# tsereda/fast-cwdm

Hardware: AMD Instinct MI355X
Metric: denoising-steps/sec on 8-ch 128^3 volumes (1000-step DDPM, i2i cWDM) (higher is better)
Workload: dtype bf16; 1 GPU; config2: BraTS 3->1 conditional synthesis, 1xMI355X per replica, 128^3 subbands, 1000-step DDPM (direct linear schedule); model=UNetModel run.sh (mc 64, mult 1,2,2,4,4, 2 res blocks, 81.5M params), global_batch=1, seq_len=2097152, parallelism=replicas1

## Files before the change

### fast-cwdm_amd/csrc/conv3d_sg.hip

```cpp
#include <algorithm>
#include <atomic>
#include <cstdlib>
#include <type_traits>

#include "conv3d_v4.hpp"

namespace cwdm {

typedef float sg_f32x4 __attribute__((ext_vector_type(4)));

template <int BX, int BY, int PAD>
struct SGCfg {
  static constexpr int HX = BX + 2 * PAD, HY = BY + 2 * PAD, HZ = 4 + 2 * PAD, HV = HX * HY * HZ;
  static constexpr int PCS = (HV + 63) / 64;
  static constexpr int HVP = PCS * 64;
  static constexpr int SUB = HVP * 32;
  static constexpr int BUF = 2 * SUB;
  static constexpr int WBUF = 27 * 1024;
  static constexpr int SMEM = 2 * BUF + 2 * WBUF;
  static constexpr int LPO = 16 / BX;
  static constexpr int NR = 3 * LPO + 3;
  static_assert(BX * BY == 64, "a brick plane is 64 voxels");
};

struct SGParams {
  V4Params v;
  int ntile16;
  int parts;
  int tx, ty;
  int ksplit, kper;
  float* part;
  unsigned* count;
  int xcd;
  int diag;
  int late;
};
#ifdef CWDM_SG_DIAG
#define SG_DIAG(bit) ((q.diag & (bit)) != 0)
#else
#define SG_DIAG(bit) false
#endif

thread_local unsigned* g_sg_sync = nullptr;
constexpr int64_t kSgSyncWords = 1 << 16;

__device__ __forceinline__ void sg_mfma(sg_f32x4& acc, const u32x4& a, const u32x4& b, bf16_t*) {
  acc = __builtin_amdgcn_mfma_f32_16x16x32_bf16(__builtin_bit_cast(bf16x8, a), __builtin_bit_cast(bf16x8, b), acc, 0,
                                                0, 0);
}
__device__ __forceinline__ void sg_mfma(sg_f32x4& acc, const u32x4& a, const u32x4& b, f16_t*) {
  acc = __builtin_amdgcn_mfma_f32_16x16x32_f16(__builtin_bit_cast(f16x8, a), __builtin_bit_cast(f16x8, b), acc, 0, 0,
                                               0);
}

template <typename T, int BX, int BY, int MODE, int TAPS>
__global__ void __launch_bounds__(256) conv3d_sg_kernel(SGParams q) {
  static_assert(TAPS == 27 || TAPS == 1, "3x3x3 or 1x1");
  constexpr int PAD = TAPS == 27 ? 1 : 0;
  using C = SGCfg<BX, BY, PAD>;
  const V4Params& p = q.v;
  __shared__ __attribute__((aligned(1024))) unsigned char smem[C::SMEM];
  const int tid = threadIdx.x, lane = tid & 63, l16 = lane & 15, kq = lane >> 4;
  const int wv = __builtin_amdgcn_readfirstlane(tid >> 6);
  V4_STAMP(0);
#ifdef CWDM_CONV_STAMPS
  if (p.stamps && tid == 0) {
    p.stamps[(long long)blockIdx.x * 24 + 20] = __builtin_amdgcn_s_memrealtime();
    p.stamps[(long long)blockIdx.x * 24 + 22] = __builtin_amdgcn_s_getreg((4 << 0) | (0 << 6) | (31 << 11));
    p.stamps[(long long)blockIdx.x * 24 + 23] = __builtin_amdgcn_s_getreg((20 << 0) | (0 << 6) | (31 << 11));
  }
#endif

  int wi = blockIdx.x;
  if (q.xcd) {
    const int n = (int)gridDim.x, xj = wi & 7, q8 = n >> 3, r8 = n & 7;
    wi = (xj < r8 ? xj * (q8 + 1) : r8 * (q8 + 1) + (xj - r8) * q8) + (wi >> 3);
  }
  const int t16 = wi % q.ntile16;
  const int ks = (wi / q.ntile16) % q.ksplit;
  const int st = wi / (q.ntile16 * q.ksplit);
  const int b = st / q.parts, brick = st - b * q.parts;
  const int tx = q.tx, ty = q.ty;
  const int x0 = (brick % tx) * BX, y0 = ((brick / tx) % ty) * BY, z0 = (brick / (tx * ty)) * 4;
  const int SH = MODE == 1 ? p.H >> 1 : p.H, SW = MODE == 1 ? p.W >> 1 : p.W;
  const int nch = p.nch / 2;
  const int cb0 = ks * q.kper, cb1 = min(nch, cb0 + q.kper);

  auto issue_halo = [&](int c, int hbuf) {
    if (SG_DIAG(2)) return;
    unsigned char* hb = smem + hbuf * C::BUF;
#pragma unroll
    for (int j = 0; j < C::PCS; ++j) {
      const int pc = wv + 4 * j;
      const int sub = pc / (2 * C::PCS), blk = pc - sub * (2 * C::PCS);
      const int hv = blk * 32 + (lane >> 1);
      const int qd = 2 * sub + (lane & 1);
      if (hv >= C::HV) continue;
      int sv = -1;
// ... 8 lines not shown
      const int sc = 2 * c + (qd >> 1);
      const bool s0 = sc < p.nch0;
      const unsigned char* base = s0 ? reinterpret_cast<const unsigned char*>(p.a0) + (long long)b * p.a0_bstride
                                     : reinterpret_cast<const unsigned char*>(p.a1) + (long long)b * p.a1_bstride;
      const __amdgpu_buffer_rsrc_t rs =
          __builtin_amdgcn_make_buffer_rsrc((void*)base, (short)0, (int)(s0 ? p.a0_bytes : p.a1_bytes), 0x00020000);
      const bool cm = s0 && p.a0_cm;
      const unsigned rowb = cm ? 32u : (unsigned)(s0 ? p.ac0 : p.ac1) * 2u;
      const unsigned cofs = cm ? (unsigned)sc * (unsigned)p.a0_cvox * 32u : (unsigned)((s0 ? sc : sc - p.nch0) * 32);
      const unsigned voff = sv >= 0 ? (unsigned)sv * rowb + cofs + (unsigned)((qd & 1) * 16) : 0xFFFFFFF0u;
      __builtin_amdgcn_raw_ptr_buffer_load_lds(rs, (__attribute__((address_space(3))) void*)(hb + pc * 1024), 16, voff,
                                               0, 0, 0);
    }
  };

  const int ct64 = t16 >> 2, row = (t16 & 3) * 16 + l16;
  const unsigned wlane = (unsigned)(row * 32 + (((kq & 1) ^ ((row >> 3) & 1)) << 4));
  const __amdgpu_buffer_rsrc_t wrs = __builtin_amdgcn_make_buffer_rsrc(
      (void*)(p.aw + (long long)ct64 * p.nch * TAPS * 2048), (short)0, p.nch * TAPS * 2048, 0x00020000);
  auto issue_w = [&](int c, int wbuf) {
    if (SG_DIAG(4)) return;
    unsigned char* wb = smem + 2 * C::BUF + wbuf * C::WBUF;
    const unsigned cb = (unsigned)((2 * c + (kq >> 1)) * TAPS) * 2048u + wlane;
#pragma unroll
    for (int j = 0; j < (TAPS + 3) / 4; ++j) {
      const int t = wv + 4 * j;
      if (t < TAPS)
        __builtin_amdgcn_raw_ptr_buffer_load_lds(wrs, (__attribute__((address_space(3))) void*)(wb + t * 1024), 16,
                                                 cb + (unsigned)t * 2048u, 0, 0, 0);
    }
  };

  const int xl = l16 % BX, yl = l16 / BX;
  const int hlane = (kq >> 1) * C::SUB + (kq & 1) * 16 + ((wv * C::HY + yl) * C::HX + xl) * 32;

  sg_f32x4 acc[4];
  {
    float bi[4];
#pragma unroll
    for (int i = 0; i < 4; ++i)
      bi[i] = (p.bias && q.ksplit == 1 && !SG_DIAG(32)) ? p.bias[(long long)b * p.bias_bs + t16 * 16 + 4 * kq + i] : 0.f;
#pragma unroll
    for (int m = 0; m < 4; ++m) acc[m] = sg_f32x4{bi[0], bi[1], bi[2], bi[3]};
  }

  issue_halo(cb0, 0);
  issue_w(cb0, 0);
  asm volatile("s_waitcnt vmcnt(0)" ::: "memory");
  __builtin_amdgcn_s_barrier();
  V4_STAMP(1);
  for (int c = cb0; c < cb1; ++c) {
    const bool has_next = c + 1 < cb1;
    const int buf = (c - cb0) & 1;
    const unsigned char* hb = smem + buf * C::BUF + hlane;
    const unsigned char* wb = smem + 2 * C::BUF + buf * C::WBUF + lane * 16;
    u32x4 av[2][C::NR], aw[2][3];
    auto read_group = [&](u32x4 (&a)[C::NR], u32x4 (&w)[3], int g) {
      if (SG_DIAG(8)) return;
      const int dz = g / 3, dx = g % 3;
#pragma unroll
      for (int dy = 0; dy < 3; ++dy) w[dy] = *reinterpret_cast<const u32x4*>(wb + (dz * 9 + dy * 3 + dx) * 1024);
#pragma unroll
      for (int s = 0; s < C::NR; ++s)
        a[s] = *reinterpret_cast<const u32x4*>(hb + ((dz * C::HY + s) * C::HX + dx) * 32);
    };
    if constexpr (TAPS == 27) {
      read_group(av[0], aw[0], 0);
    } else {
#pragma unroll
      for (int s2 = 0; s2 < 4 * C::LPO; s2 += C::LPO)
        av[0][s2] = *reinterpret_cast<const u32x4*>(hb + s2 * C::HX * 32);
      aw[0][0] = *reinterpret_cast<const u32x4*>(wb);
    }
    const int late = TAPS == 27 ? q.late : 0;
    if (has_next && late == 0) {
      issue_halo(c + 1, buf ^ 1);
      issue_w(c + 1, buf ^ 1);
    }
    if constexpr (TAPS == 27) {
#pragma unroll
      for (int g = 0; g < 9; ++g) {
        if (g + 1 < 9) read_group(av[(g + 1) & 1], aw[(g + 1) & 1], g + 1);
        __builtin_amdgcn_sched_barrier(0);
#pragma unroll
        for (int dy = 0; dy < 3; ++dy)
#pragma unroll
          for (int m = 0; m < 4; ++m)
            if (!SG_DIAG(1)) sg_mfma(acc[m], aw[g & 1][dy], av[g & 1][m * C::LPO + dy], (T*)nullptr);
        __builtin_amdgcn_sched_barrier(0);
        if (has_next && late == g + 1) {
          issue_halo(c + 1, buf ^ 1);
          issue_w(c + 1, buf ^ 1);
        }
      }
    } else {
#pragma unroll
      for (int m = 0; m < 4; ++m) sg_mfma(acc[m], aw[0][0], av[0][m * C::LPO], (T*)nullptr);
    }
    if (has_next) {
      asm volatile("s_waitcnt vmcnt(0)" ::: "memory");
      __builtin_amdgcn_s_barrier();
    }
    if (c - cb0 < 8) V4_STAMP(4 + c - cb0);
  }
  V4_STAMP(12);
  if (SG_DIAG(16)) return;

  if (q.ksplit > 1 && !SG_DIAG(64)) {
    const int tile = st * q.ntile16 + t16;
    const __amdgpu_buffer_rsrc_t prs = __builtin_amdgcn_make_buffer_rsrc(
        q.part + (long long)tile * q.ksplit * 4096, (short)0, q.ksplit * 4096 * 4, 0x00020000);
    const unsigned lofs = (unsigned)(wv * 4 * 64 + lane) * 16u;
#pragma unroll
    for (int m = 0; m < 4; ++m)
      __builtin_amdgcn_raw_buffer_store_b128(__builtin_bit_cast(u32x4, acc[m]), prs,
                                             (unsigned)ks * 16384u + lofs + (unsigned)m * 1024u, 0, 16);
    asm volatile("s_waitcnt vmcnt(0)" ::: "memory");
    __syncthreads();
    unsigned* flag = reinterpret_cast<unsigned*>(smem);
    if (tid == 0)
      *flag = __hip_atomic_fetch_add(&q.count[tile], 1u, __ATOMIC_RELAXED, __HIP_MEMORY_SCOPE_AGENT);
    __syncthreads();
    V4_STAMP(13);
    if (*flag != (unsigned)(q.ksplit - 1)) {
      V4_STAMP(15);
#ifdef CWDM_CONV_STAMPS
      if (p.stamps && tid == 0) p.stamps[(long long)blockIdx.x * 24 + 21] = __builtin_amdgcn_s_memrealtime();
#endif
      return;
    }
    if (tid == 0) __hip_atomic_store(&q.count[tile], 0u, __ATOMIC_RELAXED, __HIP_MEMORY_SCOPE_AGENT);
    float bi[4];
#pragma unroll
    for (int i = 0; i < 4; ++i) bi[i] = p.bias ? p.bias[(long long)b * p.bias_bs + t16 * 16 + 4 * kq + i] : 0.f;
#pragma unroll
    for (int m = 0; m < 4; ++m) {
      sg_f32x4 sum = __builtin_bit_cast(sg_f32x4, __builtin_amdgcn_raw_buffer_load_b128(prs, lofs + m * 1024u, 0, 16));
      for (int k = 1; k < q.ksplit; ++k)
        sum += __builtin_bit_cast(sg_f32x4,
                                  __builtin_amdgcn_raw_buffer_load_b128(prs, (unsigned)k * 16384u + lofs + m * 1024u, 0, 16));
      acc[m] = sum + sg_f32x4{bi[0], bi[1], bi[2], bi[3]};
    }
    V4_STAMP(14);
  }

  const int ox = x0 + xl, oz = z0 + wv;
  const long long HW = (long long)p.H * p.W;
  float ssum[4] = {0.f, 0.f, 0.f, 0.f}, ssq[4] = {0.f, 0.f, 0.f, 0.f};
  const int co = t16 * 16 + 4 * kq;
  bool inb[4];
#pragma unroll
  for (int m = 0; m < 4; ++m) inb[m] = ox < p.W && (y0 + m * C::LPO + yl) < p.H && oz < p.D;
  uint2 rq[4];
  float4 rf[4];
  if (p.rmode >= 0) {
#pragma unroll
    for (int m = 0; m < 4; ++m) {
      const int oy = y0 + m * C::LPO + yl;
      long long rvox = ((long long)b * p.D + oz) * HW + (long long)oy * p.W + ox;
      if (p.rmode == 1)
        rvox = (((long long)b * (p.D >> 1) + (oz >> 1)) * (p.H >> 1) + (oy >> 1)) * (p.W >> 1) + (ox >> 1);
      rq[m] = uint2{0u, 0u};
      rf[m] = make_float4(0.f, 0.f, 0.f, 0.f);
      if (inb[m]) {
        if (p.out_f32) rf[m] = *reinterpret_cast<const float4*>(reinterpret_cast<const float*>(p.res) + rvox * p.cout + co);
        else rq[m] = *reinterpret_cast<const uint2*>(reinterpret_cast<const T*>(p.res) + rvox * p.cout + co);
      }
    }
  }
#pragma unroll
  for (int m = 0; m < 4; ++m) {
    const int oy = y0 + m * C::LPO + yl;
    const long long vox = ((long long)b * p.D + oz) * HW + (long long)oy * p.W + ox;
    float v[4];
#pragma unroll
    for (int i = 0; i < 4; ++i) v[i] = acc[m][i];
    if (p.rmode >= 0) {
      if (p.out_f32) {
        v[0] += rf[m].x; v[1] += rf[m].y; v[2] += rf[m].z; v[3] += rf[m].w;
      } else {
        v[0] += lo2f<T>(rq[m].x); v[1] += hi2f<T>(rq[m].x);
        v[2] += lo2f<T>(rq[m].y); v[3] += hi2f<T>(rq[m].y);
      }
    }
    if (inb[m]) {
#pragma unroll
      for (int i = 0; i < 4; ++i) {
        ssum[i] += v[i];
        ssq[i] += v[i] * v[i];
      }
      if (p.out_f32) {
        *reinterpret_cast<float4*>(reinterpret_cast<float*>(p.out) + vox * p.cout + co) = make_float4(v[0], v[1], v[2], v[3]);
      } else {
        uint2 sq;
        sq.x = pack2<T>(v[0], v[1]);
        sq.y = pack2<T>(v[2], v[3]);
        *reinterpret_cast<uint2*>(reinterpret_cast<T*>(p.out) + vox * p.cout + co) = sq;
      }
    }
  }
  if (p.stats) {
#pragma unroll
    for (int i = 0; i < 4; ++i) {
      ssum[i] = row16_sum(ssum[i]);
      ssq[i] = row16_sum(ssq[i]);
    }
    __syncthreads();
    float* R = reinterpret_cast<float*>(smem);
    if (l16 == 0) {
#pragma unroll
      for (int i = 0; i < 4; ++i) {
        R[wv * 32 + 4 * kq + i] = ssum[i];
        R[wv * 32 + 16 + 4 * kq + i] = ssq[i];
      }
    }
    __syncthreads();
    if (tid < 16) {
      float s = 0.f, s2 = 0.f;
#pragma unroll
      for (int w = 0; w < 4; ++w) {
        s += R[w * 32 + tid];
        s2 += R[w * 32 + 16 + tid];
      }
      const long long pidx = ((long long)b * q.parts + brick) * p.cout + t16 * 16 + tid;
      p.stats[pidx * 2 + 0] = s;
      p.stats[pidx * 2 + 1] = s2;
    }
  }
  V4_STAMP(15);
#ifdef CWDM_CONV_STAMPS
  if (p.stamps && tid == 0) p.stamps[(long long)blockIdx.x * 24 + 21] = __builtin_amdgcn_s_memrealtime();
#endif
}

template __global__ void conv3d_sg_kernel<bf16_t, 16, 4, 0, 27>(SGParams);
template __global__ void conv3d_sg_kernel<bf16_t, 16, 4, 1, 27>(SGParams);
template __global__ void conv3d_sg_kernel<bf16_t, 16, 4, 0, 1>(SGParams);
template __global__ void conv3d_sg_kernel<bf16_t, 8, 8, 0, 27>(SGParams);
template __global__ void conv3d_sg_kernel<bf16_t, 8, 8, 1, 27>(SGParams);
template __global__ void conv3d_sg_kernel<bf16_t, 8, 8, 0, 1>(SGParams);
template __global__ void conv3d_sg_kernel<f16_t, 16, 4, 0, 27>(SGParams);
template __global__ void conv3d_sg_kernel<f16_t, 16, 4, 1, 27>(SGParams);
template __global__ void conv3d_sg_kernel<f16_t, 16, 4, 0, 1>(SGParams);
template __global__ void conv3d_sg_kernel<f16_t, 8, 8, 0, 27>(SGParams);
template __global__ void conv3d_sg_kernel<f16_t, 8, 8, 1, 27>(SGParams);
template __global__ void conv3d_sg_kernel<f16_t, 8, 8, 0, 1>(SGParams);

thread_local bool g_sg_fp32x = false;

namespace {
bool sg_shape_ok(const cwdm_conv3d_desc* d) {
  if (g_conv_path.load(std::memory_order_relaxed) == 1) return false;
  if (!dtype_half(d->dtype) || d->accumulate || d->out1 || d->cout % 64) return false;
  if (d->out_dtype != d->dtype && !(d->out_dtype == CWDM_F32 && g_sg_fp32x)) return false;
  return d->W >= 1 && d->W < kWideMinW && d->H >= 1 && d->D >= 1;
}

struct SgGeom { int bx, tx, ty, tz; int64_t parts() const { return (int64_t)tx * ty * tz; } };
SgGeom sg_geom(const cwdm_conv3d_desc* d) {
  const int bx = d->W >= 16 ? 16 : 8, by = 64 / bx;
  return SgGeom{bx, (int)ceil_div(d->W, bx), (int)ceil_div(d->H, by), (int)ceil_div(d->D, 4)};
// ... 21 lines not shown
int sg_split_for(const cwdm_conv3d_desc* d, int cin, bool skip = false) {
  const int64_t parts = sg_geom(d).parts();
  const int64_t tiles = d->B * parts * (d->cout / 16);
  const int nch = cin / 32;
  static const int64_t target3 = env_ll("CWDM_SG_TARGET", 192);
  static const int64_t target1 = env_ll("CWDM_SG_SKIP_TARGET", target3);
  const int64_t target = skip ? target1 : target3;
  if (tiles >= target || nch < 2) return 1;
  int S = (int)std::min<int64_t>((target + tiles - 1) / tiles, nch);
  const int per = (nch + S - 1) / S;
  S = (nch + per - 1) / per;
  return (tiles * S < (1 << 16) && S > 1) ? S : 1;
}
}

int sg_ksplit(const cwdm_conv3d_desc* d) { return sg_eligible(d) ? sg_split_for(d, d->a_c0 + d->a_c1) : 1; }
int64_t ksplit_slice_voxels(const cwdm_conv3d_desc* d) {
  return sg_shape_ok(d) ? sg_geom(d).parts() * 256 : d->D * d->H * d->W;
}
int sg_skip_ksplit(const cwdm_conv3d_desc* d) { return sg_skip_eligible(d) ? sg_split_for(d, d->b_c0 + d->b_c1, true) : 1; }

int64_t sg_sync_bytes(int ksplit) { return ksplit > 1 ? kSgSyncWords * 4 : 0; }
int64_t plan_sync_bytes() { return kSgSyncWords * 4 + kV5AaWords * 4; }
unsigned* plan_aa_counters() { return g_sg_sync ? g_sg_sync + kSgSyncWords : nullptr; }

namespace {
int sg_counters(SGParams& q, void* own, hipStream_t s) {
  q.count = nullptr;
  if (q.ksplit == 1) return CWDM_OK;
  const int64_t tiles = (int64_t)q.v.B * q.parts * q.ntile16;
  CWDM_REQUIRE(tiles <= kSgSyncWords, CWDM_E_UNSUPPORTED, "conv3d (small grid): too many K-split tiles");
  if (g_sg_sync) {
    q.count = g_sg_sync;
    return CWDM_OK;
  }
  CWDM_REQUIRE(own, CWDM_E_INVALID, "conv3d (small grid): K-split counters missing");
  q.count = reinterpret_cast<unsigned*>(own);
  CWDM_HIP(hipMemsetAsync(own, 0, (size_t)((tiles * 4 + 15) & ~15LL), s));
  return CWDM_OK;
}

template <typename T>
void sg_go_t(const SGParams& q, const cwdm_conv3d_desc* d, int taps, hipStream_t s) {
  const dim3 grid((unsigned)(d->B * q.parts * q.ntile16 * q.ksplit));
  const bool w8 = sg_geom(d).bx == 8;
  if (w8 && taps == 1) {
    hipLaunchKernelGGL((conv3d_sg_kernel<T, 8, 8, 0, 1>), grid, dim3(256), 0, s, q);
  } else if (w8) {
    if (q.v.amode == 1) hipLaunchKernelGGL((conv3d_sg_kernel<T, 8, 8, 1, 27>), grid, dim3(256), 0, s, q);
    else hipLaunchKernelGGL((conv3d_sg_kernel<T, 8, 8, 0, 27>), grid, dim3(256), 0, s, q);
  } else if (taps == 1) {
    hipLaunchKernelGGL((conv3d_sg_kernel<T, 16, 4, 0, 1>), grid, dim3(256), 0, s, q);
  } else if (q.v.amode == 1) {
    hipLaunchKernelGGL((conv3d_sg_kernel<T, 16, 4, 1, 27>), grid, dim3(256), 0, s, q);
  } else {
    hipLaunchKernelGGL((conv3d_sg_kernel<T, 16, 4, 0, 27>), grid, dim3(256), 0, s, q);
  }
}

int sg_go(const SGParams& q0, const cwdm_conv3d_desc* d, int taps, double flops, hipStream_t s) {
  static const int xcd_map = env_not0("CWDM_SG_XCD");
  SGParams q = q0;
  q.xcd = xcd_map;
  static const int late = env_int("CWDM_SG_LATE", 4);
  q.late = late < 0 ? 0 : (late > 9 ? 9 : late);
#ifdef CWDM_SG_DIAG
  static const int diag = env_int("CWDM_SG_DIAGMASK", 0);
  q.diag = diag;
#endif
  prof_begin(s);
  if (d->dtype == CWDM_F16) sg_go_t<f16_t>(q, d, taps, s);
  else sg_go_t<bf16_t>(q, d, taps, s);
  prof_end(s, flops);
  CWDM_LAUNCHED();
  return CWDM_OK;
}
}

int sg_launch(const V4Params& v, const cwdm_conv3d_desc* d, void* partial, hipStream_t s) {
  SGParams q{};
  q.v = v;
  q.ntile16 = d->cout / 16;
  const SgGeom gm = sg_geom(d);
  q.parts = (int)gm.parts();
  q.tx = gm.tx; q.ty = gm.ty;
  q.ksplit = sg_ksplit(d);
  q.kper = ((d->a_c0 + d->a_c1) / 32 + q.ksplit - 1) / q.ksplit;
  q.part = reinterpret_cast<float*>(partial);
  CWDM_REQUIRE(q.ksplit == 1 || partial, CWDM_E_INVALID, "conv3d (small grid): K-split scratch missing");
  int rc;
  if ((rc = sg_counters(q, q.ksplit > 1 ? reinterpret_cast<unsigned char*>(partial) +
                                              (int64_t)q.ksplit * d->B * ksplit_slice_voxels(d) * d->cout * 4
                                        : nullptr, s)))
    return rc;
  return sg_go(q, d, 27, 2.0 * d->B * d->D * d->H * d->W * (double)d->cout * 27.0 * (d->a_c0 + d->a_c1), s);
}

int sg_skip_launch(const cwdm_conv3d_desc* d, void* out, void* partial, hipStream_t s) {
  SGParams q{};
  V4Params& p = q.v;
  const int64_t V = d->D * d->H * d->W;
  p.B = (int)d->B; p.D = (int)d->D; p.H = (int)d->H; p.W = (int)d->W;
  p.cout = d->cout; p.nct = d->cout / 64;
  p.nch0 = d->b_c0 / 16; p.nch = (d->b_c0 + d->b_c1) / 16;
  p.a0 = d->b0; p.ac0 = d->b_c0; p.a1 = d->b1; p.ac1 = d->b_c1;
  p.a0_bstride = V * d->b_c0 * 2; p.a1_bstride = V * d->b_c1 * 2;
  p.a0_bytes = (unsigned)(V * d->b_c0 * 2); p.a1_bytes = (unsigned)(V * d->b_c1 * 2);
  p.amode = 0; p.a0_cm = 0; p.a0_cvox = (int)V;
  p.aw = reinterpret_cast<const unsigned char*>(d->b_w);
  p.bias = nullptr; p.res = nullptr; p.rmode = -1;
  p.out = out; p.stats = nullptr;
  p.out_f32 = (d->out_dtype == CWDM_F32) ? 1 : 0;
  q.ntile16 = d->cout / 16;
  const SgGeom gm = sg_geom(d);
  q.parts = (int)gm.parts();
  q.tx = gm.tx; q.ty = gm.ty;
  q.ksplit = sg_skip_ksplit(d);
  q.kper = ((d->b_c0 + d->b_c1) / 32 + q.ksplit - 1) / q.ksplit;
  q.part = reinterpret_cast<float*>(partial);
  CWDM_REQUIRE(q.ksplit == 1 || partial, CWDM_E_INVALID, "conv3d (small grid): K-split scratch missing");
  int rc;
  if ((rc = sg_counters(q, q.ksplit > 1 ? reinterpret_cast<unsigned char*>(partial) +
                                              (int64_t)q.ksplit * d->B * ksplit_slice_voxels(d) * d->cout * 4
                                        : nullptr, s)))
    return rc;
  return sg_go(q, d, 1, 2.0 * d->B * V * (double)d->cout * (d->b_c0 + d->b_c1), s);
}

}
```

### fast-cwdm_amd/cwdm_hip/_lib.py

```python
import ctypes
import os

_HERE = os.path.dirname(os.path.abspath(__file__))
LIB_PATH = os.environ.get("CWDM_LIB", os.path.join(_HERE, "..", "lib", "libcwdm.so"))

CWDM_F32 = 0
CWDM_BF16 = 1
CWDM_F64 = 2
CWDM_F16 = 3

E_INVALID, E_SHAPE, E_HIP, E_WORKSPACE, E_INDEX, E_UNSUPPORTED = -1, -2, -3, -4, -5, -6

i64 = ctypes.c_int64
vp = ctypes.c_void_p
I64x3 = i64 * 3
I64x4 = i64 * 4


class SamplerArgs(ctypes.Structure):
    _fields_ = [
        ("model_out", vp), ("mo_s", I64x3),
        ("x_t", vp), ("xt_s", I64x3),
        ("x_prev", vp), ("xp_s", I64x3),
        ("noise", vp), ("nz_s", I64x3),
# ... 111 lines not shown
    "cwdm_conv3d_parts": (i64, [ctypes.c_int, i64, i64, i64, ctypes.c_int]),
    "cwdm_space_to_depth": (ctypes.c_int, [vp, ctypes.c_int, i64, i64, i64, i64, ctypes.c_int, vp, ctypes.c_int,
                                           ctypes.c_int, vp]),
    "cwdm_conv3d_pack_s2": (ctypes.c_int, [vp, ctypes.c_int, ctypes.c_int, ctypes.c_int, vp, ctypes.c_int, vp]),
    "cwdm_conv3d_s2_fold_dw": (ctypes.c_int, [vp, ctypes.c_int, ctypes.c_int, vp, ctypes.c_int, vp]),
    "cwdm_conv3d_forward": (ctypes.c_int, [ctypes.POINTER(ConvDesc), vp]),
    "cwdm_conv3d_workspace_bytes": (i64, [ctypes.POINTER(ConvDesc)]),
    "cwdm_gn_finalize": (ctypes.c_int, [vp, i64, ctypes.c_int, vp, i64, ctypes.c_int, vp, vp, ctypes.c_int, i64, i64,
                                        ctypes.c_float, vp, vp, vp]),
    "cwdm_gn_silu_pool": (ctypes.c_int, [vp, ctypes.c_int, vp, i64, i64, i64, i64, ctypes.c_int, vp, vp, vp]),
    "cwdm_gn_apply": (ctypes.c_int, [vp, ctypes.c_int, vp, ctypes.c_int, vp, i64, i64, ctypes.c_int, vp, vp]),
    "cwdm_conv3d_set_path": (ctypes.c_int, [ctypes.c_int]),
    "cwdm_debug_v5_grid": (ctypes.c_int, [ctypes.c_int]),
    "cwdm_debug_v5_aa": (ctypes.c_int, [ctypes.c_int]),
    "cwdm_debug_up_phase": (ctypes.c_int, [ctypes.c_int]),
    "cwdm_debug_stats_wg": (i64, [ctypes.c_int]),
    "cwdm_debug_v5_aa_timeout": (ctypes.c_int, [ctypes.c_int, ctypes.c_int]),
    "cwdm_device_status": (ctypes.c_int, [ctypes.c_int]),
    "cwdm_debug_gn_fin_apply": (ctypes.c_int, [vp, i64, ctypes.c_int, vp, i64, ctypes.c_int, vp, vp, ctypes.c_int,
                                               i64, i64, ctypes.c_float, vp, vp, ctypes.c_int, vp, vp, vp, vp]),
    "cwdm_debug_head2": (ctypes.c_int, [ctypes.c_int]),
    "cwdm_debug_pw_lt": (ctypes.c_int, [ctypes.c_int]),
    "cwdm_debug_conv_stamps": (ctypes.c_int, [vp]),
    "cwdm_conv3d_wgrad": (ctypes.c_int, [ctypes.POINTER(WgradDesc), vp]),
    "cwdm_conv3d_wgrad_workspace_bytes": (i64, [ctypes.c_int, ctypes.c_int, ctypes.c_int]),
    "cwdm_gn_silu_bwd_workspace_bytes": (i64, [ctypes.c_int, i64, i64, i64, i64]),
    "cwdm_gn_silu_bwd": (ctypes.c_int, [vp, ctypes.c_int, vp, ctypes.c_int, vp, ctypes.c_int, vp, vp, vp,
                                        ctypes.c_int, i64, i64, i64, i64, ctypes.c_int, vp, ctypes.c_int, vp,
                                        ctypes.c_int, vp, vp, vp, i64, vp]),
    "cwdm_resample_add": (ctypes.c_int, [vp, vp, ctypes.c_int, i64, i64, i64, i64, ctypes.c_int, ctypes.c_int,
# ... 114 lines not shown
```

### include/cwdm.h

```cpp
#ifndef CWDM_H_
#define CWDM_H_

#include <stddef.h>
#include <stdint.h>

#ifdef __cplusplus
extern "C" {
#endif

typedef struct ihipStream_t* cwdm_stream_t;

enum {
  CWDM_F32 = 0,
  CWDM_BF16 = 1,
  CWDM_F64 = 2,
  CWDM_F16 = 3
};

enum {
  CWDM_OK = 0,
  CWDM_E_INVALID = -1,
  CWDM_E_SHAPE = -2,
  CWDM_E_HIP = -3,
  CWDM_E_WORKSPACE = -4,
// ... 135 lines not shown
                     int64_t B, int64_t voxels, float eps,
                     float* scale_shift, float* mean_rstd ,
                     cwdm_stream_t stream);

int cwdm_gn_silu_pool(const void* x, int C, const float* gn, int64_t B, int64_t d, int64_t h, int64_t w,
                      int dtype, void* out_h, void* out_x, cwdm_stream_t stream);

int cwdm_conv3d_set_path(int path);

int cwdm_debug_v5_grid(int n);

int cwdm_debug_v5_aa(int on);

int cwdm_debug_up_phase(int on);

int64_t cwdm_debug_stats_wg(int on);

int cwdm_debug_v5_aa_timeout(int extra, int spin);

enum { CWDM_DEV_E_AA_TIMEOUT = 1 };
int cwdm_device_status(int clear);

int cwdm_debug_gn_fin_apply(const float* stats0, int64_t parts0, int c0, const float* stats1, int64_t parts1,
                            int c1, const float* gamma, const float* beta, int groups, int64_t B, int64_t voxels,
                            float eps, const void* x0, const void* x1, int dtype, float* scale_shift,
                            float* mean_rstd, void* out_cm, cwdm_stream_t stream);

int cwdm_debug_head2(int mode);

int cwdm_debug_pw_lt(int on);
// ... 102 lines not shown
```

Before: 67.56 denoising-steps/s.

## Add wide small-grid conv forms covering two bricks and/or two channel tiles

Templates the small-grid 3x3x3 conv kernel on NB (bricks along y) and NT (16-channel output tiles per workgroup), so one halo fill feeds more output rows and one weight fill feeds more channels. When LDS cannot hold double buffers, it falls back to single buffering with an extra barrier. A host-side cost model picks the form and K-split per layer. It is on by default through CWDM_SG_WIDE. The aim is more MFMA work per LDS fill and fewer, fuller workgroups on small-grid layers, at the cost of more registers (lower occupancy), fewer workgroups, and possible serialization when single-buffered.

Result: no change. 68.03 denoising-steps/s (median of 6 runs) (+0.7%).

```diff
diff --git a/fast-cwdm_amd/csrc/conv3d_sg.hip b/fast-cwdm_amd/csrc/conv3d_sg.hip
--- a/fast-cwdm_amd/csrc/conv3d_sg.hip
+++ b/fast-cwdm_amd/csrc/conv3d_sg.hip
@@ -9,18 +9,25 @@
 
 typedef float sg_f32x4 __attribute__((ext_vector_type(4)));
 
-template <int BX, int BY, int PAD>
+template <int BX, int BY, int PAD, int NB = 1, int NT = 1>
 struct SGCfg {
-  static constexpr int HX = BX + 2 * PAD, HY = BY + 2 * PAD, HZ = 4 + 2 * PAD, HV = HX * HY * HZ;
+  static constexpr int HX = BX + 2 * PAD, HY = BY * NB + 2 * PAD, HZ = 4 + 2 * PAD, HV = HX * HY * HZ;
   static constexpr int PCS = (HV + 63) / 64;
   static constexpr int HVP = PCS * 64;
   static constexpr int SUB = HVP * 32;
   static constexpr int BUF = 2 * SUB;
-  static constexpr int WBUF = 27 * 1024;
-  static constexpr int SMEM = 2 * BUF + 2 * WBUF;
+  static constexpr int WB1 = 27 * 1024;
+  static constexpr int WBUF = NT * WB1;
+  static constexpr int LDS = 160 * 1024;
+  static constexpr int HBN = 2 * BUF + WBUF <= LDS ? 2 : 1;
+  static constexpr int WBN = HBN * BUF + 2 * WBUF <= LDS ? 2 : 1;
+  static constexpr int SMEM = HBN * BUF + WBN * WBUF;
   static constexpr int LPO = 16 / BX;
-  static constexpr int NR = 3 * LPO + 3;
+  static constexpr int NOP = 4 * NB;
+  static constexpr int NR = (NOP - 1) * LPO + 3;
   static_assert(BX * BY == 64, "a brick plane is 64 voxels");
+  static_assert((NB == 1 || NB == 2) && (NT == 1 || NT == 2), "1 or 2 bricks x 1 or 2 channel tiles");
+  static_assert(PAD == 1 || (NB == 1 && NT == 1), "the wide forms are 27-tap only");
 };
 
 struct SGParams {
@@ -28,6 +35,7 @@
   int ntile16;
   int parts;
   int tx, ty;
+  int typ, tparts;
   int ksplit, kper;
   float* part;
   unsigned* count;
@@ -53,11 +61,12 @@
                                                0);
 }
 
-template <typename T, int BX, int BY, int MODE, int TAPS>
+template <typename T, int BX, int BY, int MODE, int TAPS, int NB = 1, int NT = 1>
 __global__ void __launch_bounds__(256) conv3d_sg_kernel(SGParams q) {
   static_assert(TAPS == 27 || TAPS == 1, "3x3x3 or 1x1");
   constexpr int PAD = TAPS == 27 ? 1 : 0;
-  using C = SGCfg<BX, BY, PAD>;
+  using C = SGCfg<BX, BY, PAD, NB, NT>;
+  constexpr int NOP = C::NOP;
   const V4Params& p = q.v;
   __shared__ __attribute__((aligned(1024))) unsigned char smem[C::SMEM];
   const int tid = threadIdx.x, lane = tid & 63, l16 = lane & 15, kq = lane >> 4;
@@ -79,9 +88,10 @@
   const int t16 = wi % q.ntile16;
   const int ks = (wi / q.ntile16) % q.ksplit;
   const int st = wi / (q.ntile16 * q.ksplit);
-  const int b = st / q.parts, brick = st - b * q.parts;
+  const int b = st / q.tparts, tb = st - b * q.tparts;
   const int tx = q.tx, ty = q.ty;
-  const int x0 = (brick % tx) * BX, y0 = ((brick / tx) % ty) * BY, z0 = (brick / (tx * ty)) * 4;
+  const int xb = tb % tx, yb = ((tb / tx) % q.typ) * NB, zb = tb / (tx * q.typ);
+  const int x0 = xb * BX, y0 = yb * BY, z0 = zb * 4;
   const int SH = MODE == 1 ? p.H >> 1 : p.H, SW = MODE == 1 ? p.W >> 1 : p.W;
   const int nch = p.nch / 2;
   const int cb0 = ks * q.kper, cb1 = min(nch, cb0 + q.kper);
@@ -120,34 +130,39 @@
     }
   };
 
-  const int ct64 = t16 >> 2, row = (t16 & 3) * 16 + l16;
+  const int ct64 = (t16 * NT) >> 2, row = ((t16 * NT) & 3) * 16 + l16;
   const unsigned wlane = (unsigned)(row * 32 + (((kq & 1) ^ ((row >> 3) & 1)) << 4));
   const __amdgpu_buffer_rsrc_t wrs = __builtin_amdgcn_make_buffer_rsrc(
       (void*)(p.aw + (long long)ct64 * p.nch * TAPS * 2048), (short)0, p.nch * TAPS * 2048, 0x00020000);
   auto issue_w = [&](int c, int wbuf) {
     if (SG_DIAG(4)) return;
-    unsigned char* wb = smem + 2 * C::BUF + wbuf * C::WBUF;
+    unsigned char* wb = smem + C::HBN * C::BUF + wbuf * C::WBUF;
     const unsigned cb = (unsigned)((2 * c + (kq >> 1)) * TAPS) * 2048u + wlane;
 #pragma unroll
-    for (int j = 0; j < (TAPS + 3) / 4; ++j) {
-      const int t = wv + 4 * j;
-      if (t < TAPS)
-        __builtin_amdgcn_raw_ptr_buffer_load_lds(wrs, (__attribute__((address_space(3))) void*)(wb + t * 1024), 16,
-                                                 cb + (unsigned)t * 2048u, 0, 0, 0);
-    }
+    for (int nt = 0; nt < NT; ++nt)
+#pragma unroll
+      for (int j = 0; j < (TAPS + 3) / 4; ++j) {
+        const int t = wv + 4 * j;
+        if (t < TAPS)
+          __builtin_amdgcn_raw_ptr_buffer_load_lds(wrs, (__attribute__((address_space(3))) void*)(wb + nt * C::WB1 + t * 1024),
+                                                   16, cb + (unsigned)(nt * 512) + (unsigned)t * 2048u, 0, 0, 0);
+      }
   };
 
   const int xl = l16 % BX, yl = l16 / BX;
   const int hlane = (kq >> 1) * C::SUB + (kq & 1) * 16 + ((wv * C::HY + yl) * C::HX + xl) * 32;
 
-  sg_f32x4 acc[4];
-  {
+  sg_f32x4 acc[NT][NOP];
+#pragma unroll
+  for (int nt = 0; nt < NT; ++nt) {
     float bi[4];
 #pragma unroll
     for (int i = 0; i < 4; ++i)
-      bi[i] = (p.bias && q.ksplit == 1 && !SG_DIAG(32)) ? p.bias[(long long)b * p.bias_bs + t16 * 16 + 4 * kq + i] : 0.f;
-#pragma unroll
-    for (int m = 0; m < 4; ++m) acc[m] = sg_f32x4{bi[0], bi[1], bi[2], bi[3]};
+      bi[i] = (p.bias && q.ksplit == 1 && !SG_DIAG(32))
+                  ? p.bias[(long long)b * p.bias_bs + (t16 * NT + nt) * 16 + 4 * kq + i]
+                  : 0.f;
+#pragma unroll
+    for (int m = 0; m < NOP; ++m) acc[nt][m] = sg_f32x4{bi[0], bi[1], bi[2], bi[3]};
   }
 
   issue_halo(cb0, 0);
@@ -158,14 +173,18 @@
   for (int c = cb0; c < cb1; ++c) {
     const bool has_next = c + 1 < cb1;
     const int buf = (c - cb0) & 1;
-    const unsigned char* hb = smem + buf * C::BUF + hlane;
-    const unsigned char* wb = smem + 2 * C::BUF + buf * C::WBUF + lane * 16;
-    u32x4 av[2][C::NR], aw[2][3];
-    auto read_group = [&](u32x4 (&a)[C::NR], u32x4 (&w)[3], int g) {
+    const int hbuf = C::HBN == 2 ? buf : 0, wbuf = C::WBN == 2 ? buf : 0;
+    const unsigned char* hb = smem + hbuf * C::BUF + hlane;
+    const unsigned char* wb = smem + C::HBN * C::BUF + wbuf * C::WBUF + lane * 16;
+    u32x4 av[2][C::NR], aw[2][NT][3];
+    auto read_group = [&](u32x4 (&a)[C::NR], u32x4 (&w)[NT][3], int g) {
       if (SG_DIAG(8)) return;
       const int dz = g / 3, dx = g % 3;
 #pragma unroll
-      for (int dy = 0; dy < 3; ++dy) w[dy] = *reinterpret_cast<const u32x4*>(wb + (dz * 9 + dy * 3 + dx) * 1024);
+      for (int nt = 0; nt < NT; ++nt)
+#pragma unroll
+        for (int dy = 0; dy < 3; ++dy)
+          w[nt][dy] = *reinterpret_cast<const u32x4*>(wb + nt * C::WB1 + (dz * 9 + dy * 3 + dx) * 1024);
 #pragma unroll
       for (int s = 0; s < C::NR; ++s)
         a[s] = *reinterpret_cast<const u32x4*>(hb + ((dz * C::HY + s) * C::HX + dx) * 32);
@@ -176,12 +195,12 @@
 #pragma unroll
       for (int s2 = 0; s2 < 4 * C::LPO; s2 += C::LPO)
         av[0][s2] = *reinterpret_cast<const u32x4*>(hb + s2 * C::HX * 32);
-      aw[0][0] = *reinterpret_cast<const u32x4*>(wb);
+      aw[0][0][0] = *reinterpret_cast<const u32x4*>(wb);
     }
     const int late = TAPS == 27 ? q.late : 0;
     if (has_next && late == 0) {
-      issue_halo(c + 1, buf ^ 1);
-      issue_w(c + 1, buf ^ 1);
+      if constexpr (C::HBN == 2) issue_halo(c + 1, buf ^ 1);
+      if constexpr (C::WBN == 2) issue_w(c + 1, buf ^ 1);
     }
     if constexpr (TAPS == 27) {
 #pragma unroll
@@ -191,17 +210,26 @@
 #pragma unroll
         for (int dy = 0; dy < 3; ++dy)
 #pragma unroll
-          for (int m = 0; m < 4; ++m)
-            if (!SG_DIAG(1)) sg_mfma(acc[m], aw[g & 1][dy], av[g & 1][m * C::LPO + dy], (T*)nullptr);
+          for (int m = 0; m < NOP; ++m)
+#pragma unroll
+            for (int nt = 0; nt < NT; ++nt)
+              if (!SG_DIAG(1)) sg_mfma(acc[nt][m], aw[g & 1][nt][dy], av[g & 1][m * C::LPO + dy], (T*)nullptr);
         __builtin_amdgcn_sched_barrier(0);
         if (has_next && late == g + 1) {
-          issue_halo(c + 1, buf ^ 1);
-          issue_w(c + 1, buf ^ 1);
+          if constexpr (C::HBN == 2) issue_halo(c + 1, buf ^ 1);
+          if constexpr (C::WBN == 2) issue_w(c + 1, buf ^ 1);
         }
       }
     } else {
 #pragma unroll
-      for (int m = 0; m < 4; ++m) sg_mfma(acc[m], aw[0][0], av[0][m * C::LPO], (T*)nullptr);
+      for (int m = 0; m < 4; ++m) sg_mfma(acc[0][m], aw[0][0][0], av[0][m * C::LPO], (T*)nullptr);
+    }
+    if constexpr (C::HBN == 1 || C::WBN == 1) {
+      if (has_next) {
+        __builtin_amdgcn_s_barrier();
+        if constexpr (C::HBN == 1) issue_halo(c + 1, 0);
+        if constexpr (C::WBN == 1) issue_w(c + 1, 0);
+      }
     }
     if (has_next) {
       asm volatile("s_waitcnt vmcnt(0)" ::: "memory");
@@ -213,14 +241,17 @@
   if (SG_DIAG(16)) return;
 
   if (q.ksplit > 1 && !SG_DIAG(64)) {
+    constexpr int SLW = NB * NT * 4096;
     const int tile = st * q.ntile16 + t16;
     const __amdgpu_buffer_rsrc_t prs = __builtin_amdgcn_make_buffer_rsrc(
-        q.part + (long long)tile * q.ksplit * 4096, (short)0, q.ksplit * 4096 * 4, 0x00020000);
-    const unsigned lofs = (unsigned)(wv * 4 * 64 + lane) * 16u;
-#pragma unroll
-    for (int m = 0; m < 4; ++m)
-      __builtin_amdgcn_raw_buffer_store_b128(__builtin_bit_cast(u32x4, acc[m]), prs,
-                                             (unsigned)ks * 16384u + lofs + (unsigned)m * 1024u, 0, 16);
+        q.part + (long long)tile * q.ksplit * SLW, (short)0, q.ksplit * SLW * 4, 0x00020000);
+    const unsigned lofs = (unsigned)(wv * NT * NOP * 64 + lane) * 16u;
+#pragma unroll
+    for (int nt = 0; nt < NT; ++nt)
+#pragma unroll
+      for (int m = 0; m < NOP; ++m)
+        __builtin_amdgcn_raw_buffer_store_b128(__builtin_bit_cast(u32x4, acc[nt][m]), prs,
+                                               (unsigned)ks * (SLW * 4u) + lofs + (unsigned)(nt * NOP + m) * 1024u, 0, 16);
     asm volatile("s_waitcnt vmcnt(0)" ::: "memory");
     __syncthreads();
     unsigned* flag = reinterpret_cast<unsigned*>(smem);
@@ -236,101 +267,134 @@
       return;
     }
     if (tid == 0) __hip_atomic_store(&q.count[tile], 0u, __ATOMIC_RELAXED, __HIP_MEMORY_SCOPE_AGENT);
-    float bi[4];
-#pragma unroll
-    for (int i = 0; i < 4; ++i) bi[i] = p.bias ? p.bias[(long long)b * p.bias_bs + t16 * 16 + 4 * kq + i] : 0.f;
-#pragma unroll
-    for (int m = 0; m < 4; ++m) {
-      sg_f32x4 sum = __builtin_bit_cast(sg_f32x4, __builtin_amdgcn_raw_buffer_load_b128(prs, lofs + m * 1024u, 0, 16));
-      for (int k = 1; k < q.ksplit; ++k)
-        sum += __builtin_bit_cast(sg_f32x4,
-                                  __builtin_amdgcn_raw_buffer_load_b128(prs, (unsigned)k * 16384u + lofs + m * 1024u, 0, 16));
-      acc[m] = sum + sg_f32x4{bi[0], bi[1], bi[2], bi[3]};
+    for (int k = 0; k < q.ksplit; ++k) {
+      sg_f32x4 sl[NT][NOP];
+#pragma unroll
+      for (int nt = 0; nt < NT; ++nt)
+#pragma unroll
+        for (int m = 0; m < NOP; ++m)
+          sl[nt][m] = __builtin_bit_cast(
+              sg_f32x4, __builtin_amdgcn_raw_buffer_load_b128(
+                            prs, (unsigned)k * (SLW * 4u) + lofs + (unsigned)(nt * NOP + m) * 1024u, 0, 16));
+#pragma unroll
+      for (int nt = 0; nt < NT; ++nt)
+#pragma unroll
+        for (int m = 0; m < NOP; ++m) acc[nt][m] = k == 0 ? sl[nt][m] : acc[nt][m] + sl[nt][m];
+    }
+#pragma unroll
+    for (int nt = 0; nt < NT; ++nt) {
+      float bi[4];
+#pragma unroll
+      for (int i = 0; i < 4; ++i)
+        bi[i] = p.bias ? p.bias[(long long)b * p.bias_bs + (t16 * NT + nt) * 16 + 4 * kq + i] : 0.f;
+#pragma unroll
+      for (int m = 0; m < NOP; ++m) acc[nt][m] += sg_f32x4{bi[0], bi[1], bi[2], bi[3]};
     }
     V4_STAMP(14);
   }
 
   const int ox = x0 + xl, oz = z0 + wv;
   const long long HW = (long long)p.H * p.W;
-  float ssum[4] = {0.f, 0.f, 0.f, 0.f}, ssq[4] = {0.f, 0.f, 0.f, 0.f};
-  const int co = t16 * 16 + 4 * kq;
-  bool inb[4];
-#pragma unroll
-  for (int m = 0; m < 4; ++m) inb[m] = ox < p.W && (y0 + m * C::LPO + yl) < p.H && oz < p.D;
-  uint2 rq[4];
-  float4 rf[4];
-  if (p.rmode >= 0) {
-#pragma unroll
-    for (int m = 0; m < 4; ++m) {
+  float ssum[NB][NT][4], ssq[NB][NT][4];
+#pragma unroll
+  for (int nb = 0; nb < NB; ++nb)
+#pragma unroll
+    for (int nt = 0; nt < NT; ++nt)
+#pragma unroll
+      for (int i = 0; i < 4; ++i) ssum[nb][nt][i] = ssq[nb][nt][i] = 0.f;
+  bool inb[NOP];
+#pragma unroll
+  for (int m = 0; m < NOP; ++m) inb[m] = ox < p.W && (y0 + m * C::LPO + yl) < p.H && oz < p.D;
+#pragma unroll
+  for (int nt = 0; nt < NT; ++nt) {
+    const int co = (t16 * NT + nt) * 16 + 4 * kq;
+    uint2 rq[NOP];
+    float4 rf[NOP];
+    if (p.rmode >= 0) {
+#pragma unroll
+      for (int m = 0; m < NOP; ++m) {
+        const int oy = y0 + m * C::LPO + yl;
+        long long rvox = ((long long)b * p.D + oz) * HW + (long long)oy * p.W + ox;
+        if (p.rmode == 1)
+          rvox = (((long long)b * (p.D >> 1) + (oz >> 1)) * (p.H >> 1) + (oy >> 1)) * (p.W >> 1) + (ox >> 1);
+        rq[m] = uint2{0u, 0u};
+        rf[m] = make_float4(0.f, 0.f, 0.f, 0.f);
+        if (inb[m]) {
+          if (p.out_f32) rf[m] = *reinterpret_cast<const float4*>(reinterpret_cast<const float*>(p.res) + rvox * p.cout + co);
+          else rq[m] = *reinterpret_cast<const uint2*>(reinterpret_cast<const T*>(p.res) + rvox * p.cout + co);
+        }
+      }
+    }
+#pragma unroll
+    for (int m = 0; m < NOP; ++m) {
       const int oy = y0 + m * C::LPO + yl;
-      long long rvox = ((long long)b * p.D + oz) * HW + (long long)oy * p.W + ox;
-      if (p.rmode == 1)
-        rvox = (((long long)b * (p.D >> 1) + (oz >> 1)) * (p.H >> 1) + (oy >> 1)) * (p.W >> 1) + (ox >> 1);
-      rq[m] = uint2{0u, 0u};
-      rf[m] = make_float4(0.f, 0.f, 0.f, 0.f);
+      const long long vox = ((long long)b * p.D + oz) * HW + (long long)oy * p.W + ox;
+      float v[4];
+#pragma unroll
+      for (int i = 0; i < 4; ++i) v[i] = acc[nt][m][i];
+      if (p.rmode >= 0) {
+        if (p.out_f32) {
+          v[0] += rf[m].x; v[1] += rf[m].y; v[2] += rf[m].z; v[3] += rf[m].w;
+        } else {
+          v[0] += lo2f<T>(rq[m].x); v[1] += hi2f<T>(rq[m].x);
+          v[2] += lo2f<T>(rq[m].y); v[3] += hi2f<T>(rq[m].y);
+        }
+      }
       if (inb[m]) {
-        if (p.out_f32) rf[m] = *reinterpret_cast<const float4*>(reinterpret_cast<const float*>(p.res) + rvox * p.cout + co);
-        else rq[m] = *reinterpret_cast<const uint2*>(reinterpret_cast<const T*>(p.res) + rvox * p.cout + co);
-      }
-    }
-  }
-#pragma unroll
-  for (int m = 0; m < 4; ++m) {
-    const int oy = y0 + m * C::LPO + yl;
-    const long long vox = ((long long)b * p.D + oz) * HW + (long long)oy * p.W + ox;
-    float v[4];
-#pragma unroll
-    for (int i = 0; i < 4; ++i) v[i] = acc[m][i];
-    if (p.rmode >= 0) {
-      if (p.out_f32) {
-        v[0] += rf[m].x; v[1] += rf[m].y; v[2] += rf[m].z; v[3] += rf[m].w;
-      } else {
-        v[0] += lo2f<T>(rq[m].x); v[1] += hi2f<T>(rq[m].x);
-        v[2] += lo2f<T>(rq[m].y); v[3] += hi2f<T>(rq[m].y);
-      }
-    }
-    if (inb[m]) {
-#pragma unroll
-      for (int i = 0; i < 4; ++i) {
-        ssum[i] += v[i];
-        ssq[i] += v[i] * v[i];
-      }
-      if (p.out_f32) {
-        *reinterpret_cast<float4*>(reinterpret_cast<float*>(p.out) + vox * p.cout + co) = make_float4(v[0], v[1], v[2], v[3]);
-      } else {
-        uint2 sq;
-        sq.x = pack2<T>(v[0], v[1]);
-        sq.y = pack2<T>(v[2], v[3]);
-        *reinterpret_cast<uint2*>(reinterpret_cast<T*>(p.out) + vox * p.cout + co) = sq;
+#pragma unroll
+        for (int i = 0; i < 4; ++i) {
+          ssum[m / 4][nt][i] += v[i];
+          ssq[m / 4][nt][i] += v[i] * v[i];
+        }
+        if (p.out_f32) {
+          *reinterpret_cast<float4*>(reinterpret_cast<float*>(p.out) + vox * p.cout + co) = make_float4(v[0], v[1], v[2], v[3]);
+        } else {
+          uint2 sq;
+          sq.x = pack2<T>(v[0], v[1]);
+          sq.y = pack2<T>(v[2], v[3]);
+          *reinterpret_cast<uint2*>(reinterpret_cast<T*>(p.out) + vox * p.cout + co) = sq;
+        }
       }
     }
   }
   if (p.stats) {
 #pragma unroll
-    for (int i = 0; i < 4; ++i) {
-      ssum[i] = row16_sum(ssum[i]);
-      ssq[i] = row16_sum(ssq[i]);
-    }
+    for (int nb = 0; nb < NB; ++nb)
+#pragma unroll
+      for (int nt = 0; nt < NT; ++nt)
+#pragma unroll
+        for (int i = 0; i < 4; ++i) {
+          ssum[nb][nt][i] = row16_sum(ssum[nb][nt][i]);
+          ssq[nb][nt][i] = row16_sum(ssq[nb][nt][i]);
+        }
     __syncthreads();
     float* R = reinterpret_cast<float*>(smem);
     if (l16 == 0) {
 #pragma unroll
-      for (int i = 0; i < 4; ++i) {
-        R[wv * 32 + 4 * kq + i] = ssum[i];
-        R[wv * 32 + 16 + 4 * kq + i] = ssq[i];
-      }
+      for (int nb = 0; nb < NB; ++nb)
+#pragma unroll
+        for (int nt = 0; nt < NT; ++nt)
+#pragma unroll
+          for (int i = 0; i < 4; ++i) {
+            R[((wv * NB + nb) * NT + nt) * 32 + 4 * kq + i] = ssum[nb][nt][i];
+            R[((wv * NB + nb) * NT + nt) * 32 + 16 + 4 * kq + i] = ssq[nb][nt][i];
+          }
     }
     __syncthreads();
-    if (tid < 16) {
+    if (tid < 16 * NB * NT) {
+      const int ch = tid & 15, u = tid >> 4, nb = u / NT, nt = u - nb * NT;
       float s = 0.f, s2 = 0.f;
 #pragma unroll
       for (int w = 0; w < 4; ++w) {
-        s += R[w * 32 + tid];
-        s2 += R[w * 32 + 16 + tid];
-      }
-      const long long pidx = ((long long)b * q.parts + brick) * p.cout + t16 * 16 + tid;
-      p.stats[pidx * 2 + 0] = s;
-      p.stats[pidx * 2 + 1] = s2;
+        s += R[(w * NB * NT + u) * 32 + ch];
+        s2 += R[(w * NB * NT + u) * 32 + 16 + ch];
+      }
+      if (yb + nb < ty) {
+        const int brick = (zb * ty + yb + nb) * tx + xb;
+        const long long pidx = ((long long)b * q.parts + brick) * p.cout + (t16 * NT + nt) * 16 + ch;
+        p.stats[pidx * 2 + 0] = s;
+        p.stats[pidx * 2 + 1] = s2;
+      }
     }
   }
   V4_STAMP(15);
@@ -351,6 +415,19 @@
 template __global__ void conv3d_sg_kernel<f16_t, 8, 8, 0, 27>(SGParams);
 template __global__ void conv3d_sg_kernel<f16_t, 8, 8, 1, 27>(SGParams);
 template __global__ void conv3d_sg_kernel<f16_t, 8, 8, 0, 1>(SGParams);
+#define CWDM_SG_WIDE_INST(T, BX, BY, MODE)                                     \
+  template __global__ void conv3d_sg_kernel<T, BX, BY, MODE, 27, 1, 2>(SGParams); \
+  template __global__ void conv3d_sg_kernel<T, BX, BY, MODE, 27, 2, 1>(SGParams); \
+  template __global__ void conv3d_sg_kernel<T, BX, BY, MODE, 27, 2, 2>(SGParams);
+CWDM_SG_WIDE_INST(bf16_t, 16, 4, 0)
+CWDM_SG_WIDE_INST(bf16_t, 16, 4, 1)
+CWDM_SG_WIDE_INST(bf16_t, 8, 8, 0)
+CWDM_SG_WIDE_INST(bf16_t, 8, 8, 1)
+CWDM_SG_WIDE_INST(f16_t, 16, 4, 0)
+CWDM_SG_WIDE_INST(f16_t, 16, 4, 1)
+CWDM_SG_WIDE_INST(f16_t, 8, 8, 0)
+CWDM_SG_WIDE_INST(f16_t, 8, 8, 1)
+#undef CWDM_SG_WIDE_INST
 
 thread_local bool g_sg_fp32x = false;
 
@@ -402,9 +479,67 @@
 }
 }
 
-int sg_ksplit(const cwdm_conv3d_desc* d) { return sg_eligible(d) ? sg_split_for(d, d->a_c0 + d->a_c1) : 1; }
+constexpr int kSgForms = 4;
+constexpr int kSgFormNB[kSgForms] = {1, 1, 2, 2}, kSgFormNT[kSgForms] = {1, 2, 1, 2};
+std::atomic<int> g_sg_wide{-1};
+std::atomic<int> g_sg_wide_last{0};
+namespace {
+struct SgForm { int idx, nb, nt, S; };
+
+int64_t sg_form_tiles(const cwdm_conv3d_desc* d, int nb, int nt) {
+  const SgGeom gm = sg_geom(d);
+  return d->B * gm.tx * ceil_div(gm.ty, nb) * gm.tz * (d->cout / (16 * nt));
+}
+
+double sg_form_cost(const cwdm_conv3d_desc* d, int nb, int nt, int S) {
+  const int bx = sg_geom(d).bx, by = 64 / bx, nch = (d->a_c0 + d->a_c1) / 32;
+  const int64_t hv = (int64_t)(bx + 2) * (by * nb + 2) * 6;
+  const double fill = (double)ceil_div(hv, 64) * 64 * 64 + nt * 27648.0;
+  const double slice = S > 1 ? nb * nt * 16384.0 : 0.0;
+  const double rounds = (double)ceil_div(sg_form_tiles(d, nb, nt) * S, (int64_t)256);
+  return rounds * (ceil_div(nch, S) * fill + slice) + 0.5 * S * slice + (S > 1 ? 65536.0 : 0.0);
+}
+
+SgForm sg_form_for(const cwdm_conv3d_desc* d) {
+  const int cin = d->a_c0 + d->a_c1, nch = cin / 32;
+  const SgForm narrow{0, 1, 1, sg_split_for(d, cin)};
+  static const int wide = env_int("CWDM_SG_WIDE", 1);
+  const int fcode = g_sg_wide.load(std::memory_order_relaxed);
+  const int forced = fcode < 0 ? -1 : fcode & 3, fS = fcode < 0 ? 0 : fcode >> 2;
+  if (d->out_dtype == CWDM_F32 || (forced < 0 && wide == 0)) return narrow;
+  if (fS > 0) {
+    const int nb = kSgFormNB[forced], nt = kSgFormNT[forced];
+    const int per = (int)ceil_div(nch, std::min(fS, nch)), S = (int)ceil_div(nch, per);
+    return SgForm{forced, nb, nt, sg_form_tiles(d, nb, nt) * S < kSgSyncWords ? S : 1};
+  }
+  if (forced == 0) return narrow;
+  SgForm best = narrow;
+  double cbest = forced > 0 ? 1e300 : sg_form_cost(d, 1, 1, narrow.S);
+  for (int f = 1; f < kSgForms; ++f) {
+    if (forced > 0 && f != forced) continue;
+    const int nb = kSgFormNB[f], nt = kSgFormNT[f];
+    const int64_t tiles = sg_form_tiles(d, nb, nt);
+    for (int S = 1; S <= nch; ++S) {
+      if ((nch + S - 1) / S * (S - 1) >= nch) continue;
+      if (S > 1 && tiles * S >= kSgSyncWords) break;
+      const double c = sg_form_cost(d, nb, nt, S);
+      if (c < cbest) {
+        best = SgForm{f, nb, nt, S};
+        cbest = c;
+      }
+    }
+  }
+  return best;
+}
+}
+
+int sg_ksplit(const cwdm_conv3d_desc* d) { return sg_eligible(d) ? sg_form_for(d).S : 1; }
 int64_t ksplit_slice_voxels(const cwdm_conv3d_desc* d) {
-  return sg_shape_ok(d) ? sg_geom(d).parts() * 256 : d->D * d->H * d->W;
+  if (!sg_shape_ok(d)) return d->D * d->H * d->W;
+  if (!sg_eligible(d)) return sg_geom(d).parts() * 256;
+  const SgGeom gm = sg_geom(d);
+  const int nb = sg_form_for(d).nb;
+  return (int64_t)gm.tx * ceil_div(gm.ty, nb) * gm.tz * nb * 256;
 }
 int sg_skip_ksplit(const cwdm_conv3d_desc* d) { return sg_skip_eligible(d) ? sg_split_for(d, d->b_c0 + d->b_c1, true) : 1; }
 
@@ -416,7 +551,7 @@
 int sg_counters(SGParams& q, void* own, hipStream_t s) {
   q.count = nullptr;
   if (q.ksplit == 1) return CWDM_OK;
-  const int64_t tiles = (int64_t)q.v.B * q.parts * q.ntile16;
+  const int64_t tiles = (int64_t)q.v.B * q.tparts * q.ntile16;
   CWDM_REQUIRE(tiles <= kSgSyncWords, CWDM_E_UNSUPPORTED, "conv3d (small grid): too many K-split tiles");
   if (g_sg_sync) {
     q.count = g_sg_sync;
@@ -428,11 +563,23 @@
   return CWDM_OK;
 }
 
+template <typename T, int BX, int BY, int MODE>
+void sg_go_wide(const SGParams& q, int form, dim3 grid, hipStream_t s) {
+  if (form == 1) hipLaunchKernelGGL((conv3d_sg_kernel<T, BX, BY, MODE, 27, 1, 2>), grid, dim3(256), 0, s, q);
+  else if (form == 2) hipLaunchKernelGGL((conv3d_sg_kernel<T, BX, BY, MODE, 27, 2, 1>), grid, dim3(256), 0, s, q);
+  else hipLaunchKernelGGL((conv3d_sg_kernel<T, BX, BY, MODE, 27, 2, 2>), grid, dim3(256), 0, s, q);
+}
+
 template <typename T>
-void sg_go_t(const SGParams& q, const cwdm_conv3d_desc* d, int taps, hipStream_t s) {
-  const dim3 grid((unsigned)(d->B * q.parts * q.ntile16 * q.ksplit));
+void sg_go_t(const SGParams& q, const cwdm_conv3d_desc* d, int taps, int form, hipStream_t s) {
+  const dim3 grid((unsigned)(d->B * q.tparts * q.ntile16 * q.ksplit));
   const bool w8 = sg_geom(d).bx == 8;
-  if (w8 && taps == 1) {
+  if (form > 0) {
+    if (w8 && q.v.amode == 1) sg_go_wide<T, 8, 8, 1>(q, form, grid, s);
+    else if (w8) sg_go_wide<T, 8, 8, 0>(q, form, grid, s);
+    else if (q.v.amode == 1) sg_go_wide<T, 16, 4, 1>(q, form, grid, s);
+    else sg_go_wide<T, 16, 4, 0>(q, form, grid, s);
+  } else if (w8 && taps == 1) {
     hipLaunchKernelGGL((conv3d_sg_kernel<T, 8, 8, 0, 1>), grid, dim3(256), 0, s, q);
   } else if (w8) {
     if (q.v.amode == 1) hipLaunchKernelGGL((conv3d_sg_kernel<T, 8, 8, 1, 27>), grid, dim3(256), 0, s, q);
@@ -446,7 +593,7 @@
   }
 }
 
-int sg_go(const SGParams& q0, const cwdm_conv3d_desc* d, int taps, double flops, hipStream_t s) {
+int sg_go(const SGParams& q0, const cwdm_conv3d_desc* d, int taps, int form, double flops, hipStream_t s) {
   static const int xcd_map = env_not0("CWDM_SG_XCD");
   SGParams q = q0;
   q.xcd = xcd_map;
@@ -457,8 +604,8 @@
   q.diag = diag;
 #endif
   prof_begin(s);
-  if (d->dtype == CWDM_F16) sg_go_t<f16_t>(q, d, taps, s);
-  else sg_go_t<bf16_t>(q, d, taps, s);
+  if (d->dtype == CWDM_F16) sg_go_t<f16_t>(q, d, taps, form, s);
+  else sg_go_t<bf16_t>(q, d, taps, form, s);
   prof_end(s, flops);
   CWDM_LAUNCHED();
   return CWDM_OK;
@@ -468,12 +615,16 @@
 int sg_launch(const V4Params& v, const cwdm_conv3d_desc* d, void* partial, hipStream_t s) {
   SGParams q{};
   q.v = v;
-  q.ntile16 = d->cout / 16;
+  const SgForm f = sg_form_for(d);
+  q.ntile16 = d->cout / (16 * f.nt);
   const SgGeom gm = sg_geom(d);
   q.parts = (int)gm.parts();
   q.tx = gm.tx; q.ty = gm.ty;
-  q.ksplit = sg_ksplit(d);
+  q.typ = (int)ceil_div(gm.ty, f.nb);
+  q.tparts = gm.tx * q.typ * gm.tz;
+  q.ksplit = f.S;
   q.kper = ((d->a_c0 + d->a_c1) / 32 + q.ksplit - 1) / q.ksplit;
+  g_sg_wide_last.store(f.idx + 4 * f.S, std::memory_order_relaxed);
   q.part = reinterpret_cast<float*>(partial);
   CWDM_REQUIRE(q.ksplit == 1 || partial, CWDM_E_INVALID, "conv3d (small grid): K-split scratch missing");
   int rc;
@@ -481,7 +632,7 @@
                                               (int64_t)q.ksplit * d->B * ksplit_slice_voxels(d) * d->cout * 4
                                         : nullptr, s)))
     return rc;
-  return sg_go(q, d, 27, 2.0 * d->B * d->D * d->H * d->W * (double)d->cout * 27.0 * (d->a_c0 + d->a_c1), s);
+  return sg_go(q, d, 27, f.idx, 2.0 * d->B * d->D * d->H * d->W * (double)d->cout * 27.0 * (d->a_c0 + d->a_c1), s);
 }
 
 int sg_skip_launch(const cwdm_conv3d_desc* d, void* out, void* partial, hipStream_t s) {
@@ -503,6 +654,7 @@
   const SgGeom gm = sg_geom(d);
   q.parts = (int)gm.parts();
   q.tx = gm.tx; q.ty = gm.ty;
+  q.typ = gm.ty; q.tparts = q.parts;
   q.ksplit = sg_skip_ksplit(d);
   q.kper = ((d->b_c0 + d->b_c1) / 32 + q.ksplit - 1) / q.ksplit;
   q.part = reinterpret_cast<float*>(partial);
@@ -512,7 +664,12 @@
                                               (int64_t)q.ksplit * d->B * ksplit_slice_voxels(d) * d->cout * 4
                                         : nullptr, s)))
     return rc;
-  return sg_go(q, d, 1, 2.0 * d->B * V * (double)d->cout * (d->b_c0 + d->b_c1), s);
-}
-
-}
+  return sg_go(q, d, 1, 0, 2.0 * d->B * V * (double)d->cout * (d->b_c0 + d->b_c1), s);
+}
+
+}
+
+extern "C" int cwdm_debug_sg_wide(int form) {
+  if (form == -2) return cwdm::g_sg_wide_last.load(std::memory_order_relaxed);
+  return cwdm::g_sg_wide.exchange(form < 0 ? -1 : form);
+}
diff --git a/fast-cwdm_amd/cwdm_hip/_lib.py b/fast-cwdm_amd/cwdm_hip/_lib.py
--- a/fast-cwdm_amd/cwdm_hip/_lib.py
+++ b/fast-cwdm_amd/cwdm_hip/_lib.py
@@ -149,6 +149,7 @@
     "cwdm_debug_v5_grid": (ctypes.c_int, [ctypes.c_int]),
     "cwdm_debug_v5_aa": (ctypes.c_int, [ctypes.c_int]),
     "cwdm_debug_up_phase": (ctypes.c_int, [ctypes.c_int]),
+    "cwdm_debug_sg_wide": (ctypes.c_int, [ctypes.c_int]),
     "cwdm_debug_stats_wg": (i64, [ctypes.c_int]),
     "cwdm_debug_v5_aa_timeout": (ctypes.c_int, [ctypes.c_int, ctypes.c_int]),
     "cwdm_device_status": (ctypes.c_int, [ctypes.c_int]),
diff --git a/include/cwdm.h b/include/cwdm.h
--- a/include/cwdm.h
+++ b/include/cwdm.h
@@ -173,6 +173,8 @@
 
 int cwdm_debug_up_phase(int on);
 
+int cwdm_debug_sg_wide(int form);
+
 int64_t cwdm_debug_stats_wg(int on);
 
 int cwdm_debug_v5_aa_timeout(int extra, int spin);
```
